# DixianZhu/deBWT

Measured on NVIDIA B200. Metric: bwt_build_throughput, higher is better.
Workload: dtype u64

## Files before the change

debwt_b200/csrc/api.cu:

```cuda
#include <algorithm>
#include <cstring>
#include <map>
#include <mutex>
#include <string>
#include <tuple>
#include <vector>

#include "../../include/debwt_b200.h"
#include "../../include/debwt_b200_dev.h"
#include "radix_sort.cuh"
#include "stages.cuh"
#include "special.cuh"
#include "ctx.cuh"
#include "dist_kernels.cuh"

namespace debwt {

static thread_local std::string g_err;
unsigned g_launches = 0;
unsigned long long g_launches_total = 0;
void set_error(const std::string& msg) { g_err = msg; }

#define FAIL(msg)            \
    do {                     \
// ... 298 lines not shown
    mark();

    u64 *d_ka = nullptr, *d_kb = nullptr;
    if (dalloc(pool, &d_ka, nk + 2) || dalloc(pool, &d_kb, nk + 2)) return -1;
    if (k_extract(d_text, n, d_seps, R, d_ka, st)) return -1;
    mark();

    void* d_sortws = nullptr;
    if (pool.alloc(&d_sortws, sort_workspace_bytes(nk, c->sort_cfg))) return -1;
    SortWorkspace ws;
    sort_workspace_bind(ws, d_sortws, nk, c->sort_cfg);
    int sweeps = 0;
    ws.ev_sweep_begin = c->ev[11]; ws.ev_sweep_end = c->ev[12]; ws.sweeps_out = &sweeps;
    const unsigned launches_before_sort = g_launches;
    u64* d_keys = nullptr;
    KeyIndex ki;
    ki.bits = key_index_bits(nk);
    if (dalloc(pool, &ki.idx, (1ull << ki.bits) + 2) || k_key_index_init(ki, st)) return -1;
    bool index_marked = false;
    ws.key_index = ki.idx; ws.key_index_bits = ki.bits; ws.key_index_done = &index_marked;
    const bool text_hist = text_digit_hist_applies(n, R);
    if (text_hist && (radix_sort_clear(ws, st) || k_text_digit_hist(d_text, n, d_seps, R, ws.hist, st))) return -1;
    if (radix_sort_u64(d_ka, d_kb, nk, ws, st, &d_keys, text_hist)) return -1;
    S.sort_launches = g_launches - launches_before_sort;
    S.sort_sweeps = (u32)sweeps;
    pool.adopt(d_keys == d_ka ? d_kb : d_ka, (nk + 2) * 8);
    pool.adopt(d_sortws, sort_workspace_bytes(nk, c->sort_cfg));
    u32 h_err[2] = {0, 0};
    CUDA_TRY(cudaMemcpyAsync(h_err, d_err, 8, cudaMemcpyDeviceToHost, st));
    mark();

    u16* d_gmask = nullptr;
    if (dalloc(pool, &d_gmask, nk + 2)) return -1;
    CUDA_TRY(cudaMemsetAsync(d_gmask, 0, (nk + 2) * 2, st));
    if (k_key_index_finish(d_keys, nk, ki, index_marked, st)) return -1;
    if (k_mark_edges(d_keys, nk, ki, d_gmask, st)) return -1;
    if (k_mark_heads_tails(d_text, d_seps, R, d_keys, nk, ki, d_gmask, st)) return -1;
    void* d_brws = nullptr; u64* d_tot = nullptr;
    if (pool.alloc(&d_brws, branch_workspace_bytes(nk)) || dalloc(pool, &d_tot, 4)) return -1;
    if (k_branch_count(d_keys, nk, d_gmask, true, d_brws, d_tot, st)) return -1;
    u64 h_tot[2] = {0, 0};
    CUDA_TRY(cudaMemcpyAsync(h_tot, d_tot, 16, cudaMemcpyDeviceToHost, st));
    CUDA_TRY(cudaStreamSynchronize(st));
    if (h_err[0]) FAIL(c->resolve_ambiguous ? "input contains a symbol that is neither a base nor an IUPAC ambiguity code"
                                            : "input contains a symbol other than A, C, G, T (either case)");
    if (h_err[1] != R) FAIL("input contains '#' or '$' inside a record (they are reserved for the record separators)");
    BranchTable bt;
    bt.n_branch = h_tot[0]; bt.n_blue = h_tot[1];
    S.n_branch = bt.n_branch; S.n_blue = bt.n_blue;
    {
        int bits = 8;
        while (bits < 27 && (1ull << bits) < 2 * bt.n_branch) ++bits;
        bt.bits = bits;
    }
    if (dalloc(pool, &bt.kmer, bt.n_branch + 1) || dalloc(pool, &bt.head, bt.n_branch + 1) ||
        dalloc(pool, &bt.blue, bt.n_branch + 2) || dalloc(pool, &bt.cursor, bt.n_branch + 1) ||
        dalloc(pool, &bt.bidx, BranchTable::index_words(bt.bits)))
        return -1;
    CUDA_TRY(cudaMemsetAsync(bt.cursor, 0, (bt.n_branch + 1) * 4, st));
    if (k_branch_write(d_keys, nk, d_gmask, d_brws, bt, st)) return -1;
    {
        const u32 m32 = (u32)bt.n_blue;
        CUDA_TRY(cudaMemcpyAsync(bt.blue + bt.n_branch, &m32, 4, cudaMemcpyHostToDevice, st));
    }
    if (k_branch_index(bt, st)) return -1;
    int id_bits = 1;
    while (id_bits < 64 && (bt.n_branch >> id_bits)) ++id_bits;
    const bool group_by_sort = id_bits <= 28 && n < (1ull << 32) && bt.n_blue > 1 &&
                               c->blue_grouping == 2;
    bt.hbits = BranchTable::hash_bits(bt.n_branch);
    bt.hmode = group_by_sort ? 0 : 1;
    if (dalloc(pool, &bt.hslots, 1ull << bt.hbits) || k_branch_hash(bt, st)) return -1;
    mark();
// ... 422 lines not shown
    if (s.get(&d_k, n + 2) || s.get(&d_km, n + 2) || s.get(&d_ct, n + 2) || s.get(&d_tot, 2)) return -1;
    CUDA_TRY(cudaMalloc(&d_ws, rle_workspace_bytes(n)));
    s.ptrs.push_back(d_ws);
    CUDA_TRY(cudaMemcpyAsync(d_k, sorted, n * 8, cudaMemcpyHostToDevice, s.st));
    if (k_rle(d_k, n, d_km, d_ct, d_ws, d_tot, s.st)) return -1;
    u64 d = 0;
    CUDA_TRY(cudaMemcpyAsync(&d, d_tot, 8, cudaMemcpyDeviceToHost, s.st));
    CUDA_TRY(cudaStreamSynchronize(s.st));
    CUDA_TRY(cudaMemcpyAsync(kmers_out, d_km, d * 8, cudaMemcpyDeviceToHost, s.st));
    CUDA_TRY(cudaMemcpyAsync(counts_out, d_ct, d * 8, cudaMemcpyDeviceToHost, s.st));
    CUDA_TRY(cudaStreamSynchronize(s.st));
    if (n_distinct_out) *n_distinct_out = d;
    return 0;
}

int debwt_k_group_masks(int device, const char* text, uint64_t n, const uint64_t* seps, uint64_t R, uint16_t* masks_out) {
    if (check_seps(seps, R, n)) return -1;
    Scratch s;
    if (open_scratch(s, device)) return -1;
    const u64 nk = n - 32 * R;
    u8* d_a; u64 *d_w, *d_s, *d_ka, *d_kb; u32* d_e; u16* d_g; void* d_ws;
    KeyIndex ki;
    ki.bits = key_index_bits(nk);
    if (s.get(&d_a, n + 64) || s.get(&d_w, text_words(n)) || s.get(&d_e, 4) || s.get(&d_s, R) || s.get(&d_ka, nk + 2) ||
        s.get(&d_kb, nk + 2) || s.get(&d_g, nk + 2) || s.get(&ki.idx, (1ull << ki.bits) + 2))
        return -1;
    CUDA_TRY(cudaMalloc(&d_ws, sort_workspace_bytes(nk, 0)));
    s.ptrs.push_back(d_ws);
    SortWorkspace ws;
    sort_workspace_bind(ws, d_ws, nk, 0);
    CUDA_TRY(cudaMemcpyAsync(d_a, text, n, cudaMemcpyHostToDevice, s.st));
    CUDA_TRY(cudaMemcpyAsync(d_s, seps, R * 8, cudaMemcpyHostToDevice, s.st));
    CUDA_TRY(cudaMemsetAsync(d_e, 0, 16, s.st));
    CUDA_TRY(cudaMemsetAsync(d_g, 0, (nk + 2) * 2, s.st));
    u64* d_keys = nullptr;
    if (k_pack(d_a, n, d_w, d_e, s.st) || k_extract(d_w, n, d_s, R, d_ka, s.st) ||
        radix_sort_u64(d_ka, d_kb, nk, ws, s.st, &d_keys) || k_build_key_index(d_keys, nk, ki, s.st) ||
        k_mark_edges(d_keys, nk, ki, d_g, s.st) || k_mark_heads_tails(d_w, d_s, R, d_keys, nk, ki, d_g, s.st) ||
        k_propagate(d_keys, nk, d_g, s.st))
        return -1;
    CUDA_TRY(cudaMemcpyAsync(masks_out, d_g, nk * 2, cudaMemcpyDeviceToHost, s.st));
    CUDA_TRY(cudaStreamSynchronize(s.st));
    return 0;
}


int debwt_k_codes(int device, const char* text, uint64_t n, const uint64_t* seps, uint64_t R, uint8_t* codes_out, uint64_t codes_cap,
                  uint64_t* n_codes_out, uint64_t* blue_head_out, uint64_t* blue_spindex_out, uint8_t* blue_prev_out, uint64_t blue_cap,
                  uint64_t* n_blue_out) {
    debwt_ctx* c = nullptr;
    if (debwt_create(&c, device)) return -1;
    c->cap.on = true;
    int rc = debwt_set_text(c, text, n, seps, R);
    if (!rc) rc = debwt_build(c, 32);
    if (!rc) {
        const auto& q = c->cap;
        if (n_codes_out) *n_codes_out = q.n_codes;
        if (n_blue_out) *n_blue_out = q.blue.size();
        if (q.n_codes > codes_cap || q.blue.size() > blue_cap) { set_error("debwt_k_codes: output buffers too small"); rc = -1; }
    }
    if (!rc) {
        const auto& q = c->cap;
        for (u64 i = 0; i < q.n_codes; ++i) {
            u8 code = (u8)((q.codes[i >> 5] >> (2 * (31 - (i & 31)))) & 3ull);
            if ((q.sep[i >> 5] >> (i & 31)) & 1u) code = i == q.dollar_index ? 5 : 4;
            codes_out[i] = code;
        }
        for (u64 b = 0; b < q.seg_kmer.size(); ++b)
            for (u32 e = q.seg_off[b]; e < q.seg_off[b + 1]; ++e) {
                blue_head_out[e] = q.seg_head[b];
                blue_spindex_out[e] = q.blue[e] >> 4;
                blue_prev_out[e] = (u8)(q.blue[e] & 15ull);
// ... 105 lines not shown
```

debwt_b200/csrc/stages.cu:

```cuda
#include "stages.cuh"

#include <cstdlib>
#include "special.cuh"
#include "stages_dev.cuh"
#include "dist_kernels.cuh"

namespace debwt {

namespace {

constexpr int TPB = 256;
inline unsigned grid_for(u64 work, int per_block) { return (unsigned)((work + per_block - 1) / per_block); }

constexpr int SCAN_ITEMS = 16;
constexpr int SCAN_TILE = TPB * SCAN_ITEMS;

template <bool POPC>
__device__ __forceinline__ u32 scan_f(u32 v) { return POPC ? (u32)__popc(v) : v; }

template <bool POPC>
__global__ void __launch_bounds__(TPB) scan_reduce_kernel(const u32* __restrict__ in, u64 m, u32* __restrict__ part) {
    __shared__ u32 sm[40];
    const u64 base = (u64)blockIdx.x * SCAN_TILE;
    u32 s = 0;
// ... 348 lines not shown
    void* scan_ws = p;
    p += (scan_workspace_bytes(nt) + 7) & ~(size_t)7;
    u64* starts = reinterpret_cast<u64*>(p);
    rle_count_kernel<<<(unsigned)nt, TPB, 0, st>>>(sorted, n, tile_cnt);
    if (scan_exclusive_u32(tile_cnt, tile_ex, nt, false, scan_ws, d_total, st)) return -1;
    rle_write_kernel<<<(unsigned)nt, TPB, 0, st>>>(sorted, n, tile_ex, kmers, starts);
    u64 d = 0;
    CUDA_TRY(cudaMemcpyAsync(&d, d_total, 8, cudaMemcpyDeviceToHost, st));
    CUDA_TRY(cudaStreamSynchronize(st));
    diff_kernel<<<grid_for(d, TPB), TPB, 0, st>>>(starts, d, n, counts);
    DEBWT_COUNT(3);
    CUDA_TRY(cudaGetLastError());
    return 0;
}

namespace {

__global__ void __launch_bounds__(TPB) key_index_mark_kernel(const u64* __restrict__ k, u64 n, KeyIndex ki) {
    const u64 i = (u64)blockIdx.x * TPB + threadIdx.x;
    if (i >= n) return;
    const int sh = 64 - ki.bits;
    const u64 cur = k[i] >> sh;
    if (i == 0 || (k[i - 1] >> sh) != cur) ki.idx[cur] = (u32)i;
}

__global__ void __launch_bounds__(TPB) key_index_fill_kernel(const u64* __restrict__ k, u64 n, KeyIndex ki) {
    const u64 t = (u64)blockIdx.x * TPB + threadIdx.x;
    const u64 nb = 1ull << ki.bits;
    if (t > nb) return;
    if (t == nb) { ki.idx[t] = (u32)n; return; }
    if (ki.idx[t] == 0xFFFFFFFFu) ki.idx[t] = (u32)lower_bound_u64(k, 0, n, t << (64 - ki.bits));
}

constexpr int ME_ROWS = 4;

__device__ __forceinline__ void edge_rows(const u64* __restrict__ k, u64 n, const KeyIndex& ki, u16* __restrict__ gmask, u64 base,
                                          u64 limit) {
    u64 key[ME_ROWS], lo[ME_ROWS], hi[ME_ROWS];
    bool act[ME_ROWS];
#pragma unroll
    for (int j = 0; j < ME_ROWS; ++j) {
        const u64 i = base + (u64)j * TPB;
        act[j] = i < limit;
        key[j] = act[j] ? k[i] : 0;
        if (act[j] && i > 0 && k[i - 1] == key[j]) act[j] = false;
    }
#pragma unroll
    for (int j = 0; j < ME_ROWS; ++j) {
        const u64 t = (key[j] << 2) >> (64 - ki.bits);
        lo[j] = act[j] ? ki.idx[t] : 0;
        hi[j] = act[j] ? ki.idx[t + 1] : 0;
    }
#pragma unroll
    for (int j = 0; j < ME_ROWS; ++j) {
        if (!act[j]) continue;
        const u64 q = key[j] << 2;
        const u64 hs = lower_bound_u64(k, lo[j], hi[j], q);
        if (hs < n && (k[hs] >> 2) == (q >> 2)) atomic_or_u16(gmask, hs, 1u << (u32)(key[j] >> 62));
    }
#pragma unroll
    for (int j = 0; j < ME_ROWS; ++j) {
        if (!act[j]) continue;
        const u64 i = base + (u64)j * TPB;
        atomic_or_u16(gmask, group_head(k, i), 1u << (GM_OUT_SHIFT + (u32)(key[j] & 3)));
    }
}

constexpr u64 ME_TILE = 8192;
constexpr u64 ME_CAP = 8 * ME_TILE;
struct EdgeRun { u64 begin, end; };

__global__ void __launch_bounds__(TPB) edge_bounds_kernel(const u64* __restrict__ k, u64 n, KeyIndex ki, u64 tiles,
                                                         u64* __restrict__ bounds) {
    const u64 x = (u64)blockIdx.x * TPB + threadIdx.x;
    if (x >= 4 * (tiles + 1)) return;
    const u32 c = (u32)(x / (tiles + 1));
    const u64 t = x % (tiles + 1);
    const u64 cbeg = ki.idx[(u64)c << (ki.bits - 2)];
    const u64 cend = (c == 3) ? n : (u64)ki.idx[(u64)(c + 1) << (ki.bits - 2)];
    const u64 a = t * ME_TILE;
    u64 r;
    if (a == 0) r = cbeg;
    else if (a >= n) r = cend;
    else {
        const u64 low = (k[a - 1] >> 2) + 1;
        r = (low >> 62) ? cend : indexed_lower_bound(k, ki, ((u64)c << 62) | low);
    }
    bounds[x] = r;
}

__global__ void __launch_bounds__(TPB) mark_edges_kernel(const u64* __restrict__ k, u64 n, KeyIndex ki, u16* __restrict__ gmask,
                                                        const u64* __restrict__ bounds, u64 tiles, EdgeRun* __restrict__ over,
                                                        u32* __restrict__ n_over) {
    const u32 c = blockIdx.x & 3u;
    const u64 tile = blockIdx.x >> 2;
    const u64 sb = bounds[c * (tiles + 1) + tile];
    u64 se = bounds[c * (tiles + 1) + tile + 1];
    if (se - sb > ME_CAP && se > sb) {
        if (threadIdx.x == 0) over[atomicAdd(n_over, 1u)] = EdgeRun{sb + ME_CAP, se};
        se = sb + ME_CAP;
    }
    for (u64 i0 = sb; i0 < se; i0 += (u64)TPB * ME_ROWS) edge_rows(k, n, ki, gmask, i0 + threadIdx.x, se);
}

__global__ void __launch_bounds__(TPB) mark_edges_over_kernel(const u64* __restrict__ k, u64 n, KeyIndex ki, u16* __restrict__ gmask,
                                                             const EdgeRun* __restrict__ over, const u32* __restrict__ n_over) {
    const u32 m = *n_over;
    for (u32 q = 0; q < m; ++q) {
        const EdgeRun r = over[q];
        for (u64 i0 = r.begin + (u64)blockIdx.x * (TPB * ME_ROWS); i0 < r.end; i0 += (u64)gridDim.x * (TPB * ME_ROWS))
            edge_rows(k, n, ki, gmask, i0 + threadIdx.x, r.end);
    }
}

__global__ void __launch_bounds__(TPB) mark_heads_tails_kernel(const u64* __restrict__ words, const u64* __restrict__ seps,
                                                              u64 n_rec, const u64* __restrict__ k, u64 n, KeyIndex ki,
                                                              u16* __restrict__ gmask) {
    const u64 r = (u64)blockIdx.x * TPB + threadIdx.x;
    if (r >= n_rec) return;
    const u64 start = r ? seps[r - 1] + 1 : 0;
    u64 x = text_window32(words, start) & ~3ull;
    u64 h = indexed_lower_bound(k, ki, x);
    if (h < n && (k[h] & ~3ull) == x) atomic_or_u16(gmask, h, GM_IN_SEP);
    x = text_window32(words, seps[r] - KNODE) & ~3ull;
    h = indexed_lower_bound(k, ki, x);
    if (h < n && (k[h] & ~3ull) == x) atomic_or_u16(gmask, h, GM_OUT_TAIL);
}

__global__ void __launch_bounds__(TPB) propagate_kernel(const u64* __restrict__ k, u64 n, u16* __restrict__ gmask) {
    const u64 i = (u64)blockIdx.x * TPB + threadIdx.x;
    if (i >= n || i == 0) return;
    if ((k[i - 1] >> 2) != (k[i] >> 2)) return;
    gmask[i] = gmask[group_head(k, i)];
}

constexpr int BR_ITEMS = 8;
constexpr int BR_TILE = TPB * BR_ITEMS;

template <bool WRITE, bool PROPAGATE>
__global__ void __launch_bounds__(TPB) branch_kernel(const u64* __restrict__ k, u64 n, u16* __restrict__ gmask,
                                                    u32* __restrict__ tile_nb, u32* __restrict__ tile_blue,
                                                    const u32* __restrict__ tile_nb_ex, const u32* __restrict__ tile_blue_ex,
                                                    u32* __restrict__ head_bits, BranchTable bt) {
    constexpr int NW = TPB / 32;
    __shared__ u32 s_cnt[BR_ITEMS * NW + 1], s_blue[BR_ITEMS * NW + 1];
    if (WRITE && tile_nb[blockIdx.x] == 0) return;
    const int lane = threadIdx.x & 31, warp = threadIdx.x >> 5;
// ... 59 lines not shown
            if (lane >= o) { ic += tc; ib += tb; }
        }
        const u32 ec = ic - (c0 + c1), eb = ib - (b0 + b1);
        s_cnt[2 * lane] = ec; s_cnt[2 * lane + 1] = ec + c0;
        s_blue[2 * lane] = eb; s_blue[2 * lane + 1] = eb + b0;
        if (lane == 31) {
            s_cnt[BR_ITEMS * NW] = ic; s_blue[BR_ITEMS * NW] = ib;
            if (!WRITE) { tile_nb[blockIdx.x] = ic; tile_blue[blockIdx.x] = ib; }
        }
    }
    if (!WRITE) return;
    __syncthreads();
    const u64 ob0 = tile_nb_ex[blockIdx.x];
    const u32 ol0 = tile_blue_ex[blockIdx.x];
#pragma unroll
    for (int j = 0; j < BR_ITEMS; ++j) {
        if (bal[j] == 0) continue;
        u32 inc = size[j];
#pragma unroll
        for (int o = 1; o < 32; o <<= 1) {
            const u32 t = __shfl_up_sync(0xffffffffu, inc, o);
            if (lane >= o) inc += t;
        }
        if (flags[j]) {
            const u64 i = base + (u64)j * TPB + threadIdx.x;
            const u64 ob = ob0 + s_cnt[j * NW + warp] + __popc(bal[j] & lt);
            bt.kmer[ob] = (k[i] & ~3ull) | (flags[j] & 3u);
            bt.head[ob] = (u32)i;
            bt.blue[ob] = ol0 + s_blue[j * NW + warp] + (inc - size[j]);
        }
    }
}

__global__ void __launch_bounds__(TPB) branch_index_kernel(BranchTable bt) {
    const u64 t = (u64)blockIdx.x * TPB + threadIdx.x;
    const u64 nb = 1ull << bt.bits;
    if (t > nb) return;
    bt.bidx[t] = (t == nb) ? (u32)bt.n_branch : (u32)lower_bound_u64(bt.kmer, 0, bt.n_branch, t << (64 - bt.bits));
}

__global__ void __launch_bounds__(TPB) branch_filter_kernel(BranchTable bt) {
    const u64 b = (u64)blockIdx.x * TPB + threadIdx.x;
    if (b >= bt.n_branch) return;
    const u64 f = bt.filter_of(bt.kmer[b] & ~3ull);
    atomicOr(bt.filter() + (f >> 5), 1u << (f & 31));
}

__global__ void __launch_bounds__(TPB) branch_hash_kernel(BranchTable bt) {
    const u64 b = (u64)blockIdx.x * TPB + threadIdx.x;
    if (b >= bt.n_branch) return;
    const u64 e = bt.kmer[b];
    const u64 mask = (1ull << bt.hbits) - 1;
    for (u64 h = bt.hash_of(e & ~3ull);; h = (h + 1) & mask) {
        unsigned long long* claim = reinterpret_cast<unsigned long long*>(&bt.hslots[h].x);
        if (atomicCAS(claim, 0ull, (unsigned long long)e) == 0ull) {
            bt.hslots[h].y = bt.hmode ? (u64)bt.blue[b] << 32 : b;
            return;
        }
    }
}

__global__ void __launch_bounds__(TPB) special_ins_kernel(const u64* __restrict__ k, u64 n, KeyIndex ki,
                                                         const u64* __restrict__ pads, u64 m, u64* __restrict__ ins) {
    const u64 t = (u64)blockIdx.x * TPB + threadIdx.x;
    if (t < m) ins[t] = indexed_upper_bound(k, ki, pads[t]);
}

}

int k_key_index_init(KeyIndex ki, cudaStream_t st) {
    CUDA_TRY(cudaMemsetAsync(ki.idx, 0xFF, ((1ull << ki.bits) + 1) * 4, st));
    return 0;
}

int k_key_index_finish(const u64* sorted, u64 n, KeyIndex ki, bool marked, cudaStream_t st) {
    if (n && !marked) {
        key_index_mark_kernel<<<grid_for(n, TPB), TPB, 0, st>>>(sorted, n, ki);
        DEBWT_COUNT(1);
    }
    key_index_fill_kernel<<<grid_for((1ull << ki.bits) + 1, TPB), TPB, 0, st>>>(sorted, n, ki);
    DEBWT_COUNT(1);
    CUDA_TRY(cudaGetLastError());
    return 0;
}

int k_build_key_index(const u64* sorted, u64 n, KeyIndex ki, cudaStream_t st) {
    if (k_key_index_init(ki, st)) return -1;
    return k_key_index_finish(sorted, n, ki, false, st);
}

int k_mark_edges(const u64* sorted, u64 n, KeyIndex ki, u16* gmask, cudaStream_t st) {
    if (n == 0) return 0;
    const u64 tiles = (n + ME_TILE - 1) / ME_TILE;
    const u64 cap = n / ME_CAP + 8;
    char* ws = nullptr;
    CUDA_TRY(cudaMallocAsync(reinterpret_cast<void**>(&ws), 16 + cap * sizeof(EdgeRun) + 4 * (tiles + 1) * 8, st));
    u32* n_over = reinterpret_cast<u32*>(ws);
    EdgeRun* over = reinterpret_cast<EdgeRun*>(ws + 16);
    u64* bounds = reinterpret_cast<u64*>(ws + 16 + cap * sizeof(EdgeRun));
    cudaMemsetAsync(n_over, 0, 16, st);
    edge_bounds_kernel<<<grid_for(4 * (tiles + 1), TPB), TPB, 0, st>>>(sorted, n, ki, tiles, bounds);
    mark_edges_kernel<<<(unsigned)(4 * tiles), TPB, 0, st>>>(sorted, n, ki, gmask, bounds, tiles, over, n_over);
    mark_edges_over_kernel<<<148 * 8, TPB, 0, st>>>(sorted, n, ki, gmask, over, n_over);
    DEBWT_COUNT(3);
    const cudaError_t e = cudaGetLastError();
    cudaFreeAsync(ws, st);
    if (e != cudaSuccess) { set_error(std::string("mark_edges: ") + cudaGetErrorString(e)); return -1; }
    return 0;
}

int k_mark_heads_tails(const u64* words, const u64* d_seps, u64 n_rec, const u64* sorted, u64 n, KeyIndex ki, u16* gmask,
                       cudaStream_t st) {
    mark_heads_tails_kernel<<<grid_for(n_rec, TPB), TPB, 0, st>>>(words, d_seps, n_rec, sorted, n, ki, gmask);
    DEBWT_COUNT(1);
    CUDA_TRY(cudaGetLastError());
    return 0;
}

int k_propagate(const u64* sorted, u64 n, u16* gmask, cudaStream_t st) {
    if (n == 0) return 0;
    propagate_kernel<<<grid_for(n, TPB), TPB, 0, st>>>(sorted, n, gmask);
    DEBWT_COUNT(1);
    CUDA_TRY(cudaGetLastError());
    return 0;
}

namespace {
struct BranchWs { u32 *nb, *blue, *nb_ex, *blue_ex, *head_bits; void* scan_ws; u64 nt; };
BranchWs branch_ws(void* workspace, u64 n) {
    BranchWs w;
    w.nt = (n + BR_TILE - 1) / BR_TILE;
    u32* p = reinterpret_cast<u32*>(workspace);
    w.nb = p; w.blue = p + w.nt; w.nb_ex = p + 2 * w.nt; w.blue_ex = p + 3 * w.nt;
    char* q = reinterpret_cast<char*>(p + 4 * w.nt);
    q += (8 - (reinterpret_cast<uintptr_t>(q) & 7)) & 7;
    w.scan_ws = q;
    q += (scan_workspace_bytes(w.nt + 1) + 15) & ~(size_t)15;
    w.head_bits = reinterpret_cast<u32*>(q);
    return w;
}
}

size_t branch_workspace_bytes(u64 n) {
    const u64 nt = (n + BR_TILE - 1) / BR_TILE + 1;
    return nt * 16 + 16 + scan_workspace_bytes(nt) + 32 + nt * (BR_TILE / 8);
}

int k_branch_count(const u64* sorted, u64 n, u16* gmask, bool propagate, void* workspace, u64* d_totals, cudaStream_t st) {
    BranchWs w = branch_ws(workspace, n);
    BranchTable none;
    if (propagate) branch_kernel<false, true><<<(unsigned)w.nt, TPB, 0, st>>>(sorted, n, gmask, w.nb, w.blue, nullptr, nullptr, w.head_bits, none);
    else branch_kernel<false, false><<<(unsigned)w.nt, TPB, 0, st>>>(sorted, n, gmask, w.nb, w.blue, nullptr, nullptr, w.head_bits, none);
    DEBWT_COUNT(1);
    if (scan_exclusive_u32(w.nb, w.nb_ex, w.nt, false, w.scan_ws, d_totals, st)) return -1;
    if (scan_exclusive_u32(w.blue, w.blue_ex, w.nt, false, w.scan_ws, d_totals + 1, st)) return -1;
    CUDA_TRY(cudaGetLastError());
    return 0;
}

int k_branch_write(const u64* sorted, u64 n, const u16* gmask, void* workspace, BranchTable bt, cudaStream_t st) {
    BranchWs w = branch_ws(workspace, n);
    branch_kernel<true, false><<<(unsigned)w.nt, TPB, 0, st>>>(sorted, n, const_cast<u16*>(gmask), w.nb, nullptr, w.nb_ex, w.blue_ex, w.head_bits, bt);
    DEBWT_COUNT(1);
    CUDA_TRY(cudaGetLastError());
    return 0;
}

int k_branch_index(BranchTable bt, cudaStream_t st) {
    branch_index_kernel<<<grid_for((1ull << bt.bits) + 1, TPB), TPB, 0, st>>>(bt);
    CUDA_TRY(cudaMemsetAsync(bt.filter(), 0, (1ull << (BranchTable::filter_bits(bt.bits) - 5)) * 4, st));
    if (bt.n_branch) branch_filter_kernel<<<grid_for(bt.n_branch, TPB), TPB, 0, st>>>(bt);
    DEBWT_COUNT(2);
    CUDA_TRY(cudaGetLastError());
    return 0;
}

int k_branch_hash(BranchTable bt, cudaStream_t st) {
    if (!bt.hslots) return 0;
    CUDA_TRY(cudaMemsetAsync(bt.hslots, 0, (1ull << bt.hbits) * sizeof(ulonglong2), st));
    if (bt.n_branch) branch_hash_kernel<<<grid_for(bt.n_branch, TPB), TPB, 0, st>>>(bt);
    DEBWT_COUNT(1);
    CUDA_TRY(cudaGetLastError());
    return 0;
}

namespace {
__global__ void __launch_bounds__(128) special_scan_kernel(const u64* __restrict__ words, const u64* __restrict__ seps,
                                                          u64 n_rec, const u64* __restrict__ k, u64 n_keys, KeyIndex ki,
                                                          SpecialInfo* __restrict__ out) {
    __shared__ u32 s_cnt;
    const u64 m = n_rec * 32;
    const u64 a = blockIdx.x;
    const u64 pa = seps[a >> 5] - (a & 31);
    if (threadIdx.x == 0) s_cnt = 0;
    __syncthreads();
    u32 cnt = 0;
    for (u64 b = threadIdx.x; b < m; b += blockDim.x) {
// ... 620 lines not shown
```

debwt_b200/csrc/stages.cuh:

```cuda
#pragma once
#include "common.cuh"

namespace debwt {

size_t scan_workspace_bytes(u64 m);
int scan_exclusive_u32(const u32* in, u32* out, u64 m, bool popc, void* workspace, u64* d_total, cudaStream_t st);

struct PackPolicy {
    bool resolve = false;
    u64 seed = 0;
    u64 pos_base = 0;
};
int k_pack(const u8* ascii, u64 n, u64* words, u32* d_err, cudaStream_t st, PackPolicy pol = PackPolicy());
inline u64 text_words(u64 n) { return (n + 32 + 31) / 32 + 1; }
int k_extract(const u64* words, u64 n, const u64* d_seps, u64 n_rec, u64* keys, cudaStream_t st);
int k_extract_slice(const u64* words, u64 n, u64 pos_lo, u64 pos_hi, const u64* d_seps, u64 n_rec, u64 idx_base, u64* keys,
                    cudaStream_t st);

bool text_digit_hist_applies(u64 n, u64 n_rec);
int k_text_digit_hist(const u64* words, u64 n, const u64* d_seps, u64 n_rec, u64* ghist, cudaStream_t st);

int k_rle(const u64* sorted, u64 n, u64* kmers, u64* counts, void* workspace, u64* d_total, cudaStream_t st);
size_t rle_workspace_bytes(u64 n);

struct KeyIndex {
    u32* idx = nullptr;
    int bits = 0;
};
inline int key_index_bits(u64 n) {
    int b = 8;
    while (b < 28 && (8ull << b) < n) ++b;
    return b;
}
int k_build_key_index(const u64* sorted, u64 n, KeyIndex ki, cudaStream_t st);
int k_key_index_init(KeyIndex ki, cudaStream_t st);
int k_key_index_finish(const u64* sorted, u64 n, KeyIndex ki, bool marked, cudaStream_t st);
__host__ __device__ __forceinline__ u64 indexed_lower_bound(const u64* __restrict__ k, const KeyIndex& ki, u64 q) {
    const u64 t = q >> (64 - ki.bits);
    return lower_bound_u64(k, ki.idx[t], ki.idx[t + 1], q);
}
__host__ __device__ __forceinline__ u64 indexed_upper_bound(const u64* __restrict__ k, const KeyIndex& ki, u64 q) {
    const u64 t = q >> (64 - ki.bits);
    return upper_bound_u64(k, ki.idx[t], ki.idx[t + 1], q);
}

int k_mark_edges(const u64* sorted, u64 n, KeyIndex ki, u16* gmask, cudaStream_t st);
int k_mark_heads_tails(const u64* words, const u64* d_seps, u64 n_rec, const u64* sorted, u64 n, KeyIndex ki, u16* gmask,
                       cudaStream_t st);
int k_propagate(const u64* sorted, u64 n, u16* gmask, cudaStream_t st);

struct BranchTable {
    u64 n_branch = 0;
    u64 n_blue = 0;
    u64* kmer = nullptr;
    u32* head = nullptr;
    u32* blue = nullptr;
    u32* cursor = nullptr;
    u32* bidx = nullptr;
    int bits = 0;
    ulonglong2* hslots = nullptr;
    int hbits = 0;
    int hmode = 0;
    __host__ __device__ static int hash_bits(u64 n_branch) { int b = 10; while (b < 40 && (1ull << b) < 3 * n_branch) ++b; return b; }
    __host__ __device__ u64 hash_of(u64 x) const { return ((x >> 2) * 0x9E3779B97F4A7C15ull) >> (64 - hbits); }
    __host__ __device__ u64 filter_of(u64 x) const { return ((x >> 2) * 0x9E3779B97F4A7C15ull) >> (64 - filter_bits(bits)); }
    __host__ __device__ static int filter_bits(int bits) { return bits + 3 < 30 ? bits + 3 : 30; }
    __host__ __device__ static u64 index_words(int bits) { return (1ull << bits) + 2 + (1ull << (filter_bits(bits) - 5)); }
    __host__ __device__ u32* filter() const { return bidx + (1ull << bits) + 2; }
};
size_t branch_workspace_bytes(u64 n);
int k_branch_count(const u64* sorted, u64 n, u16* gmask, bool propagate, void* workspace, u64* d_totals, cudaStream_t st);
int k_branch_write(const u64* sorted, u64 n, const u16* gmask, void* workspace, BranchTable bt, cudaStream_t st);
int k_branch_index(BranchTable bt, cudaStream_t st);
int k_branch_hash(BranchTable bt, cudaStream_t st);

int k_special_insertion(const u64* sorted, u64 n, KeyIndex ki, const u64* pads, u64 m, u64* ins, cudaStream_t st);

int k_flag_positions(const u64* words, u64 n, const u64* d_seps, u64 n_rec, BranchTable bt, u32* mo_bits, u64* blue,
                     cudaStream_t st);
int k_flag_positions_keys(const u64* words, u64 n, const u64* d_seps, u64 n_rec, BranchTable bt, int shift, u32* mo_bits,
                          u64* bkeys, u64* d_counter, cudaStream_t st);
int k_blue_keys_fix(u64* bkeys, u64 m, const u32* mo_bits, const u32* word_prefix, cudaStream_t st);
int k_blue_keys_strip(u64* bkeys, u64 m, cudaStream_t st);
int k_blue_fix_interleaved(u64* blue, u64 m, const u32* mo_bits, const u32* word_prefix, u64 n_words, u64* scratch, cudaStream_t st);
int k_patch_bits(u32* mo_bits, const u64* positions, u64 m, cudaStream_t st);
int k_emit_codes(const u64* words, u64 n, const u32* mo_bits, const u32* word_prefix, u64* sp_codes, cudaStream_t st);
int k_mark_sep_codes(const u32* mo_bits, const u32* word_prefix, const u64* positions, u64 m, u32* sp_sep,
                     u64* d_code_index_out, cudaStream_t st);
int k_blue_fix(u64* blue, u64 m, const u32* mo_bits, const u32* word_prefix, cudaStream_t st);

struct SpView {
    const u64* codes;
    const u32* sep;
    u64 dollar_index;
    u64 n_codes;
    const u32* sep_sum = nullptr;
};
int k_sort_blue(u64* blue, BranchTable bt, SpView sp, u32* d_work , cudaStream_t st);

int k_fill_case2(const u16* gmask, u64 n_keys, u64 n, const u64* spec_rows, u64 m, u64* bwt, cudaStream_t st);
int k_emit_blue(const u64* blue, BranchTable bt, const u64* spec_ins, u64 m, u64* bwt, u64* sharp_rows,
                u32* d_sharp_count, u64* dollar_row, cudaStream_t st);
int k_emit_special(const u64* spec_rows, const u8* spec_chr, u64 m, u64* bwt, cudaStream_t st);

}
// ... 1 lines not shown
```

Measured before the change: 9023.

## Fuse edge marking, head/tail flags and branch counting into tiled classify kernel

Replaces the separate mask memset, mark_edges (bounds, per-tile and overflow kernels), mark_heads_tails and branch_count propagate passes with one tile-based classify kernel. It stages each 4096-key tile in shared memory, resolves group heads with ballots and a warp prefix scan, and does the predecessor-edge lookups by searching within shared memory instead of through global atomics. Per-record separator flags come from a small pre-kernel, and cross-tile groups are handled with precomputed boundary info. This is meant to cut global atomics, redundant passes over the sorted keys and launch count. In exchange it adds considerable complexity and a large dynamic shared-memory footprint, and long runs that span tiles fall back to global searches.

```diff
diff --git a/debwt_b200/csrc/api.cu b/debwt_b200/csrc/api.cu
--- a/debwt_b200/csrc/api.cu
+++ b/debwt_b200/csrc/api.cu
@@ -354,13 +354,12 @@
 
     u16* d_gmask = nullptr;
     if (dalloc(pool, &d_gmask, nk + 2)) return -1;
-    CUDA_TRY(cudaMemsetAsync(d_gmask, 0, (nk + 2) * 2, st));
     if (k_key_index_finish(d_keys, nk, ki, index_marked, st)) return -1;
-    if (k_mark_edges(d_keys, nk, ki, d_gmask, st)) return -1;
-    if (k_mark_heads_tails(d_text, d_seps, R, d_keys, nk, ki, d_gmask, st)) return -1;
-    void* d_brws = nullptr; u64* d_tot = nullptr;
-    if (pool.alloc(&d_brws, branch_workspace_bytes(nk)) || dalloc(pool, &d_tot, 4)) return -1;
-    if (k_branch_count(d_keys, nk, d_gmask, true, d_brws, d_tot, st)) return -1;
+    void* d_brws = nullptr; void* d_clws = nullptr; u64* d_tot = nullptr;
+    if (pool.alloc(&d_brws, branch_workspace_bytes(nk)) || pool.alloc(&d_clws, classify_workspace_bytes(nk)) ||
+        dalloc(pool, &d_tot, 4))
+        return -1;
+    if (k_classify(d_text, d_seps, R, d_keys, nk, ki, d_gmask, d_clws, d_brws, d_tot, st)) return -1;
     u64 h_tot[2] = {0, 0};
     CUDA_TRY(cudaMemcpyAsync(h_tot, d_tot, 16, cudaMemcpyDeviceToHost, st));
     CUDA_TRY(cudaStreamSynchronize(st));
@@ -849,12 +848,13 @@
     CUDA_TRY(cudaMemcpyAsync(d_a, text, n, cudaMemcpyHostToDevice, s.st));
     CUDA_TRY(cudaMemcpyAsync(d_s, seps, R * 8, cudaMemcpyHostToDevice, s.st));
     CUDA_TRY(cudaMemsetAsync(d_e, 0, 16, s.st));
-    CUDA_TRY(cudaMemsetAsync(d_g, 0, (nk + 2) * 2, s.st));
+    u8 *d_brws, *d_clws;
+    u64* d_tot;
+    if (s.get(&d_brws, branch_workspace_bytes(nk)) || s.get(&d_clws, classify_workspace_bytes(nk)) || s.get(&d_tot, 4)) return -1;
     u64* d_keys = nullptr;
     if (k_pack(d_a, n, d_w, d_e, s.st) || k_extract(d_w, n, d_s, R, d_ka, s.st) ||
         radix_sort_u64(d_ka, d_kb, nk, ws, s.st, &d_keys) || k_build_key_index(d_keys, nk, ki, s.st) ||
-        k_mark_edges(d_keys, nk, ki, d_g, s.st) || k_mark_heads_tails(d_w, d_s, R, d_keys, nk, ki, d_g, s.st) ||
-        k_propagate(d_keys, nk, d_g, s.st))
+        k_classify(d_w, d_s, R, d_keys, nk, ki, d_g, d_clws, d_brws, d_tot, s.st))
         return -1;
     CUDA_TRY(cudaMemcpyAsync(masks_out, d_g, nk * 2, cudaMemcpyDeviceToHost, s.st));
     CUDA_TRY(cudaStreamSynchronize(s.st));
diff --git a/debwt_b200/csrc/stages.cu b/debwt_b200/csrc/stages.cu
--- a/debwt_b200/csrc/stages.cu
+++ b/debwt_b200/csrc/stages.cu
@@ -404,87 +404,6 @@
     if (ki.idx[t] == 0xFFFFFFFFu) ki.idx[t] = (u32)lower_bound_u64(k, 0, n, t << (64 - ki.bits));
 }
 
-constexpr int ME_ROWS = 4;
-
-__device__ __forceinline__ void edge_rows(const u64* __restrict__ k, u64 n, const KeyIndex& ki, u16* __restrict__ gmask, u64 base,
-                                          u64 limit) {
-    u64 key[ME_ROWS], lo[ME_ROWS], hi[ME_ROWS];
-    bool act[ME_ROWS];
-#pragma unroll
-    for (int j = 0; j < ME_ROWS; ++j) {
-        const u64 i = base + (u64)j * TPB;
-        act[j] = i < limit;
-        key[j] = act[j] ? k[i] : 0;
-        if (act[j] && i > 0 && k[i - 1] == key[j]) act[j] = false;
-    }
-#pragma unroll
-    for (int j = 0; j < ME_ROWS; ++j) {
-        const u64 t = (key[j] << 2) >> (64 - ki.bits);
-        lo[j] = act[j] ? ki.idx[t] : 0;
-        hi[j] = act[j] ? ki.idx[t + 1] : 0;
-    }
-#pragma unroll
-    for (int j = 0; j < ME_ROWS; ++j) {
-        if (!act[j]) continue;
-        const u64 q = key[j] << 2;
-        const u64 hs = lower_bound_u64(k, lo[j], hi[j], q);
-        if (hs < n && (k[hs] >> 2) == (q >> 2)) atomic_or_u16(gmask, hs, 1u << (u32)(key[j] >> 62));
-    }
-#pragma unroll
-    for (int j = 0; j < ME_ROWS; ++j) {
-        if (!act[j]) continue;
-        const u64 i = base + (u64)j * TPB;
-        atomic_or_u16(gmask, group_head(k, i), 1u << (GM_OUT_SHIFT + (u32)(key[j] & 3)));
-    }
-}
-
-constexpr u64 ME_TILE = 8192;
-constexpr u64 ME_CAP = 8 * ME_TILE;
-struct EdgeRun { u64 begin, end; };
-
-__global__ void __launch_bounds__(TPB) edge_bounds_kernel(const u64* __restrict__ k, u64 n, KeyIndex ki, u64 tiles,
-                                                         u64* __restrict__ bounds) {
-    const u64 x = (u64)blockIdx.x * TPB + threadIdx.x;
-    if (x >= 4 * (tiles + 1)) return;
-    const u32 c = (u32)(x / (tiles + 1));
-    const u64 t = x % (tiles + 1);
-    const u64 cbeg = ki.idx[(u64)c << (ki.bits - 2)];
-    const u64 cend = (c == 3) ? n : (u64)ki.idx[(u64)(c + 1) << (ki.bits - 2)];
-    const u64 a = t * ME_TILE;
-    u64 r;
-    if (a == 0) r = cbeg;
-    else if (a >= n) r = cend;
-    else {
-        const u64 low = (k[a - 1] >> 2) + 1;
-        r = (low >> 62) ? cend : indexed_lower_bound(k, ki, ((u64)c << 62) | low);
-    }
-    bounds[x] = r;
-}
-
-__global__ void __launch_bounds__(TPB) mark_edges_kernel(const u64* __restrict__ k, u64 n, KeyIndex ki, u16* __restrict__ gmask,
-                                                        const u64* __restrict__ bounds, u64 tiles, EdgeRun* __restrict__ over,
-                                                        u32* __restrict__ n_over) {
-    const u32 c = blockIdx.x & 3u;
-    const u64 tile = blockIdx.x >> 2;
-    const u64 sb = bounds[c * (tiles + 1) + tile];
-    u64 se = bounds[c * (tiles + 1) + tile + 1];
-    if (se - sb > ME_CAP && se > sb) {
-        if (threadIdx.x == 0) over[atomicAdd(n_over, 1u)] = EdgeRun{sb + ME_CAP, se};
-        se = sb + ME_CAP;
-    }
-    for (u64 i0 = sb; i0 < se; i0 += (u64)TPB * ME_ROWS) edge_rows(k, n, ki, gmask, i0 + threadIdx.x, se);
-}
-
-__global__ void __launch_bounds__(TPB) mark_edges_over_kernel(const u64* __restrict__ k, u64 n, KeyIndex ki, u16* __restrict__ gmask,
-                                                             const EdgeRun* __restrict__ over, const u32* __restrict__ n_over) {
-    const u32 m = *n_over;
-    for (u32 q = 0; q < m; ++q) {
-        const EdgeRun r = over[q];
-        for (u64 i0 = r.begin + (u64)blockIdx.x * (TPB * ME_ROWS); i0 < r.end; i0 += (u64)gridDim.x * (TPB * ME_ROWS))
-            edge_rows(k, n, ki, gmask, i0 + threadIdx.x, r.end);
-    }
-}
-
 __global__ void __launch_bounds__(TPB) mark_heads_tails_kernel(const u64* __restrict__ words, const u64* __restrict__ seps,
                                                               u64 n_rec, const u64* __restrict__ k, u64 n, KeyIndex ki,
                                                               u16* __restrict__ gmask) {
@@ -610,6 +529,246 @@
     }
 }
 
+constexpr int CL_TPB = 256;
+constexpr int CL_ROWS = 16;
+constexpr int CL_TILE = CL_TPB * CL_ROWS;
+constexpr int CL_SEGS = CL_TILE / 32;
+constexpr int CL_SRC = 16;
+constexpr u64 CL_CHUNK = (u64)CL_TPB * CL_SRC;
+constexpr size_t CL_SMEM = CL_TILE * 8 + CL_TILE * 4 + CL_SEGS * 4 * 2;
+static_assert(CL_TILE == 2 * BR_TILE && CL_TPB == TPB, "a classify tile holds two branch tiles");
+static_assert(CL_TILE < (1 << 13), "tile-local group ends are kept in bits 16..28 of the shared mask");
+
+__global__ void __launch_bounds__(TPB) sep_flags_kernel(const u64* __restrict__ words, const u64* __restrict__ seps, u64 n_rec,
+                                                       const u64* __restrict__ k, u64 n, KeyIndex ki, u32* __restrict__ sepf) {
+    const u64 r = (u64)blockIdx.x * TPB + threadIdx.x;
+    if (r >= n_rec) return;
+    const u64 start = r ? seps[r - 1] + 1 : 0;
+    u64 x = text_window32(words, start) & ~3ull;
+    u64 h = indexed_lower_bound(k, ki, x);
+    if (h < n && (k[h] & ~3ull) == x) atomicOr(sepf + (h >> 4), 1u << (2 * (u32)(h & 15)));
+    x = text_window32(words, seps[r] - KNODE) & ~3ull;
+    h = indexed_lower_bound(k, ki, x);
+    if (h < n && (k[h] & ~3ull) == x) atomicOr(sepf + (h >> 4), 2u << (2 * (u32)(h & 15)));
+}
+
+__global__ void __launch_bounds__(TPB) classify_bounds_kernel(const u64* __restrict__ k, u64 n, KeyIndex ki, u64 tiles,
+                                                             const u32* __restrict__ sepf, u64* __restrict__ bounds,
+                                                             u8* __restrict__ cross) {
+    const u64 x = (u64)blockIdx.x * TPB + threadIdx.x;
+    if (x >= tiles * 12) return;
+    const u64 t = x / 12;
+    const u32 s = (u32)(x % 12);
+    const u64 base = t * CL_TILE;
+    if (s < 8) {
+        const u64 last = (base + CL_TILE < n ? base + CL_TILE : n) - 1;
+        const u64 q = ((u64)(s & 3) << 62) | (k[s < 4 ? base : last] >> 2);
+        bounds[t * 8 + s] = s < 4 ? indexed_lower_bound(k, ki, q) : indexed_upper_bound(k, ki, q);
+        return;
+    }
+    const u32 y = s - 8;
+    u32 v = 0;
+    const u64 key = k[base];
+    if (t > 0 && (k[base - 1] >> 2) == (key >> 2)) {
+        const u64 q = (key & ~3ull) | y;
+        const u64 h = indexed_lower_bound(k, ki, q);
+        if (h < n && k[h] == q) v = 1u << y;
+        if (y == 0) v |= ((sepf[h >> 4] >> (2 * (u32)(h & 15))) & 3u) << 4;
+    }
+    cross[t * 4 + y] = (u8)v;
+}
+
+__device__ __forceinline__ u32 cross_mask(u32 v) {
+    v |= v >> 16;
+    v |= v >> 8;
+    return ((v & 15u) << GM_OUT_SHIFT) | ((v & 16u) ? GM_IN_SEP : 0u) | ((v & 32u) ? GM_OUT_TAIL : 0u);
+}
+
+__device__ __forceinline__ u32 smem_lower_bound(const u64* __restrict__ a, u32 lo, u32 hi, u64 q) {
+    while (lo < hi) {
+        const u32 mid = (lo + hi) >> 1;
+        if (a[mid] < q) lo = mid + 1; else hi = mid;
+    }
+    return lo;
+}
+
+__device__ __forceinline__ u32 slot_of(u32 i, const u32* __restrict__ s_hb, const int* __restrict__ s_pre) {
+    const u32 m = s_hb[i >> 5] & (0xFFFFFFFFu >> (31 - (i & 31)));
+    return m ? (i & ~31u) + 31 - __clz(m) : (u32)s_pre[i >> 5];
+}
+
+__global__ void __launch_bounds__(CL_TPB, 4) classify_kernel(const u64* __restrict__ k, u64 n, const u64* __restrict__ bounds,
+                                                            const u32* __restrict__ cross, const u32* __restrict__ sepf,
+                                                            u16* __restrict__ gmask, u32* __restrict__ tile_nb,
+                                                            u32* __restrict__ tile_blue, u32* __restrict__ head_bits, u64 br_tiles) {
+    extern __shared__ u64 s_k[];
+    u32* s_gm = reinterpret_cast<u32*>(s_k + CL_TILE);
+    u32* s_hb = s_gm + CL_TILE;
+    int* s_pre = reinterpret_cast<int*>(s_hb + CL_SEGS);
+    __shared__ u64 s_run[8];
+    __shared__ u32 s_sep[CL_TILE / 16], s_cross[2];
+    __shared__ u32 s_cnt[2][CL_TPB / 32], s_blue[2][CL_TPB / 32];
+    const int lane = threadIdx.x & 31, warp = threadIdx.x >> 5;
+    const u64 base = (u64)blockIdx.x * CL_TILE;
+    const u32 tv = (u32)(n - base < (u64)CL_TILE ? n - base : (u64)CL_TILE);
+    {
+        u64 key[CL_ROWS];
+#pragma unroll
+        for (int r = 0; r < CL_ROWS; ++r) {
+            const u32 i = r * CL_TPB + threadIdx.x;
+            key[r] = i < tv ? k[base + i] : ~0ull;
+        }
+        static_assert(CL_TILE / 16 == CL_TPB, "one word of flags per thread");
+        s_sep[threadIdx.x] = threadIdx.x * 16 < tv ? sepf[base / 16 + threadIdx.x] : 0u;
+        if (threadIdx.x < 8) s_run[threadIdx.x] = bounds[(u64)blockIdx.x * 8 + threadIdx.x];
+        if (threadIdx.x == 8) s_cross[0] = cross[blockIdx.x];
+        if (threadIdx.x == 9) s_cross[1] = base + tv < n ? cross[blockIdx.x + 1] : 0u;
+#pragma unroll
+        for (int r = 0; r < CL_ROWS; ++r) s_k[r * CL_TPB + threadIdx.x] = key[r];
+    }
+    const u64 left = base ? k[base - 1] : 0;
+    const u64 right = base + tv < n ? k[base + tv] : ~0ull;
+    __syncthreads();
+    const bool cross_right = base + tv < n && (right >> 2) == (s_k[tv - 1] >> 2);
+#pragma unroll 4
+    for (int r = 0; r < CL_ROWS; ++r) {
+        const u32 i = r * CL_TPB + threadIdx.x;
+        const u64 key = s_k[i];
+        const u64 prev = i ? s_k[i - 1] : left;
+        const bool head = i < tv && (base + i == 0 || (prev >> 2) != (key >> 2));
+        const u32 hb = __ballot_sync(0xffffffffu, head);
+        if (lane == 0) s_hb[i >> 5] = hb;
+        u32 m = 0;
+        if (head) {
+            const u32 f = (s_sep[i >> 4] >> (2 * (i & 15))) & 3u;
+            m = (1u << (GM_OUT_SHIFT + (u32)(key & 3))) | ((f & 1u) ? GM_IN_SEP : 0u) | ((f & 2u) ? GM_OUT_TAIL : 0u);
+        }
+        s_gm[i] = m;
+    }
+    __syncthreads();
+    if (warp == 0) {
+        static_assert(CL_SEGS == 4 * 32, "four warp rows per lane");
+        int last[4], m = -1;
+#pragma unroll
+        for (int j = 0; j < 4; ++j) {
+            const u32 hb = s_hb[4 * lane + j];
+            if (hb) m = (4 * lane + j) * 32 + 31 - __clz(hb);
+            last[j] = m;
+        }
+        int inc = m;
+#pragma unroll
+        for (int o = 1; o < 32; o <<= 1) {
+            const int t = __shfl_up_sync(0xffffffffu, inc, o);
+            if (lane >= o && t > inc) inc = t;
+        }
+        int ex = __shfl_up_sync(0xffffffffu, inc, 1);
+        if (lane == 0) ex = -1;
+#pragma unroll
+        for (int j = 0; j < 4; ++j) {
+            s_pre[4 * lane + j] = ex < 0 ? 0 : ex;
+            if (last[j] > ex) ex = last[j];
+        }
+    }
+    __syncthreads();
+#pragma unroll 4
+    for (int r = 0; r < CL_ROWS; ++r) {
+        const u32 i = r * CL_TPB + threadIdx.x;
+        if (i >= tv) break;
+        const u32 slot = slot_of(i, s_hb, s_pre);
+        const u64 key = s_k[i];
+        u32 add = (slot != i) ? 1u << (GM_OUT_SHIFT + (u32)(key & 3)) : 0u;
+        if (i + 1 == tv || (s_k[i + 1] >> 2) != (key >> 2)) add |= (i + 1) << 16;
+        if (i == 0 && slot == 0 && base && (left >> 2) == (key >> 2)) add |= cross_mask(s_cross[0]);
+        if (i + 1 == tv && cross_right) add |= cross_mask(s_cross[1]);
+        if (add) atomicOr(s_gm + slot, add);
+    }
+    u64 o1, o2, o3, len;
+    {
+        const u64 l0 = s_run[4] - s_run[0], l1 = s_run[5] - s_run[1], l2 = s_run[6] - s_run[2], l3 = s_run[7] - s_run[3];
+        o1 = l0; o2 = o1 + l1; o3 = o2 + l2; len = o3 + l3;
+    }
+    auto at = [&](u64 v) -> u64 {
+        return v < o1 ? s_run[0] + v : v < o2 ? s_run[1] + (v - o1) : v < o3 ? s_run[2] + (v - o2) : s_run[3] + (v - o3);
+    };
+    auto run_end = [&](u64 v) -> u64 {
+        return v < o1 ? s_run[4] : v < o2 ? s_run[5] : v < o3 ? s_run[6] : s_run[7];
+    };
+    for (u64 p0 = 0; p0 < len;) {
+        const u64 p1 = p0 + CL_CHUNK < len ? p0 + CL_CHUNK : len;
+        const u64 a = p0 + (u64)threadIdx.x * CL_SRC;
+        u64 src[CL_SRC];
+#pragma unroll
+        for (int j = 0; j < CL_SRC; ++j) src[j] = (a + j < p1) ? k[at(a + j)] : ~0ull;
+        u64 next = p1;
+        if (p1 < len && p1 != o1 && p1 != o2 && p1 != o3) {
+            const u64 x = at(p1), se = run_end(p1), v = k[x - 1];
+            if (k[x] == v) {
+                u64 lo = x, step = 1;
+                while (lo + step < se && k[lo + step] == v) { lo += step; step <<= 1; }
+                next = p1 + (upper_bound_u64(k, lo + 1, lo + step < se ? lo + step : se, v) - x);
+            }
+        }
+        if (a < p1) {
+            u64 q = src[0] << 2;
+            u32 p = smem_lower_bound(s_k, 0, tv, q);
+            if (p < tv && (s_k[p] >> 2) == (q >> 2)) atomicOr(s_gm + p, 1u << (u32)(src[0] >> 62));
+#pragma unroll
+            for (int j = 1; j < CL_SRC; ++j) {
+                if (a + j >= p1) break;
+                if (src[j] == src[j - 1]) continue;
+                const u64 q2 = src[j] << 2;
+                if (q2 < q) p = smem_lower_bound(s_k, 0, tv, q2);
+                else
+                    for (int w = 0; p < tv && s_k[p] < q2; ++w, ++p)
+                        if (w == 8) { p = smem_lower_bound(s_k, p, tv, q2); break; }
+                q = q2;
+                if (p < tv && (s_k[p] >> 2) == (q >> 2)) atomicOr(s_gm + p, 1u << (u32)(src[j] >> 62));
+            }
+        }
+        p0 = next;
+    }
+    __syncthreads();
+    u32 cnt0 = 0, cnt1 = 0, blue0 = 0, blue1 = 0;
+#pragma unroll 4
+    for (int r = 0; r < CL_ROWS; ++r) {
+        const u32 i = r * CL_TPB + threadIdx.x;
+        u32 flag = 0, size = 0;
+        if (i < tv) {
+            const u32 m = s_gm[slot_of(i, s_hb, s_pre)];
+            gmask[base + i] = (u16)m;
+            if ((s_hb[i >> 5] >> lane) & 1u) {
+                const u32 f = (gm_multi_out(m) ? 1u : 0u) | (gm_multi_in(m) ? 2u : 0u);
+                flag = f;
+                if (f & 2u) {
+                    const u32 end = (m >> 16) & 0x1FFFu;
+                    size = (end == tv && cross_right) ? (u32)(group_end(k, n, base + i) - (base + i)) : end - i;
+                }
+            }
+        }
+        const u32 bal = __ballot_sync(0xffffffffu, flag != 0);
+        const u64 row = (base + (u64)r * CL_TPB) / 32 + warp;
+        if (lane == 0 && row * 32 < br_tiles * BR_TILE) head_bits[row] = bal;
+        if (bal) {
+#pragma unroll
+            for (int o = 16; o; o >>= 1) size += __shfl_xor_sync(0xffffffffu, size, o);
+        }
+        if (r < CL_ROWS / 2) { cnt0 += __popc(bal); blue0 += size; }
+        else { cnt1 += __popc(bal); blue1 += size; }
+    }
+    if (lane == 0) {
+        s_cnt[0][warp] = cnt0; s_cnt[1][warp] = cnt1;
+        s_blue[0][warp] = blue0; s_blue[1][warp] = blue1;
+    }
+    __syncthreads();
+    if (threadIdx.x < 2) {
+        const u64 bt = (u64)blockIdx.x * 2 + threadIdx.x;
+        u32 c = 0, b = 0;
+#pragma unroll
+        for (int w = 0; w < CL_TPB / 32; ++w) { c += s_cnt[threadIdx.x][w]; b += s_blue[threadIdx.x][w]; }
+        if (bt < br_tiles) { tile_nb[bt] = c; tile_blue[bt] = b; }
+    }
+}
+
 __global__ void __launch_bounds__(TPB) branch_index_kernel(BranchTable bt) {
     const u64 t = (u64)blockIdx.x * TPB + threadIdx.x;
     const u64 nb = 1ull << bt.bits;
@@ -665,26 +824,6 @@
 int k_build_key_index(const u64* sorted, u64 n, KeyIndex ki, cudaStream_t st) {
     if (k_key_index_init(ki, st)) return -1;
     return k_key_index_finish(sorted, n, ki, false, st);
-}
-
-int k_mark_edges(const u64* sorted, u64 n, KeyIndex ki, u16* gmask, cudaStream_t st) {
-    if (n == 0) return 0;
-    const u64 tiles = (n + ME_TILE - 1) / ME_TILE;
-    const u64 cap = n / ME_CAP + 8;
-    char* ws = nullptr;
-    CUDA_TRY(cudaMallocAsync(reinterpret_cast<void**>(&ws), 16 + cap * sizeof(EdgeRun) + 4 * (tiles + 1) * 8, st));
-    u32* n_over = reinterpret_cast<u32*>(ws);
-    EdgeRun* over = reinterpret_cast<EdgeRun*>(ws + 16);
-    u64* bounds = reinterpret_cast<u64*>(ws + 16 + cap * sizeof(EdgeRun));
-    cudaMemsetAsync(n_over, 0, 16, st);
-    edge_bounds_kernel<<<grid_for(4 * (tiles + 1), TPB), TPB, 0, st>>>(sorted, n, ki, tiles, bounds);
-    mark_edges_kernel<<<(unsigned)(4 * tiles), TPB, 0, st>>>(sorted, n, ki, gmask, bounds, tiles, over, n_over);
-    mark_edges_over_kernel<<<148 * 8, TPB, 0, st>>>(sorted, n, ki, gmask, over, n_over);
-    DEBWT_COUNT(3);
-    const cudaError_t e = cudaGetLastError();
-    cudaFreeAsync(ws, st);
-    if (e != cudaSuccess) { set_error(std::string("mark_edges: ") + cudaGetErrorString(e)); return -1; }
-    return 0;
 }
 
 int k_mark_heads_tails(const u64* words, const u64* d_seps, u64 n_rec, const u64* sorted, u64 n, KeyIndex ki, u16* gmask,
@@ -741,6 +880,42 @@
     branch_kernel<true, false><<<(unsigned)w.nt, TPB, 0, st>>>(sorted, n, const_cast<u16*>(gmask), w.nb, nullptr, w.nb_ex, w.blue_ex, w.head_bits, bt);
     DEBWT_COUNT(1);
     CUDA_TRY(cudaGetLastError());
+    return 0;
+}
+
+namespace {
+struct ClassifyWs { u64* bounds; u32* sepf; u8* cross; u64 tiles; };
+ClassifyWs classify_ws(void* workspace, u64 n) {
+    ClassifyWs w;
+    w.tiles = (n + CL_TILE - 1) / CL_TILE;
+    w.bounds = reinterpret_cast<u64*>(workspace);
+    w.sepf = reinterpret_cast<u32*>(w.bounds + 8 * w.tiles);
+    w.cross = reinterpret_cast<u8*>(w.sepf + (n + 15) / 16 + 1);
+    return w;
+}
+}
+
+size_t classify_workspace_bytes(u64 n) {
+    const u64 tiles = (n + CL_TILE - 1) / CL_TILE;
+    return tiles * 64 + ((n + 15) / 16 + 1) * 4 + tiles * 4 + 64;
+}
+
+int k_classify(const u64* words, const u64* d_seps, u64 n_rec, const u64* sorted, u64 n, KeyIndex ki, u16* gmask,
+               void* cl_workspace, void* br_workspace, u64* d_totals, cudaStream_t st) {
+    BranchWs b = branch_ws(br_workspace, n);
+    if (n == 0) return scan_exclusive_u32(b.nb, b.nb_ex, 0, false, b.scan_ws, d_totals, st) ||
+                       scan_exclusive_u32(b.blue, b.blue_ex, 0, false, b.scan_ws, d_totals + 1, st);
+    ClassifyWs w = classify_ws(cl_workspace, n);
+    CUDA_TRY(cudaMemsetAsync(w.sepf, 0, ((n + 15) / 16 + 1) * 4, st));
+    if (n_rec) sep_flags_kernel<<<grid_for(n_rec, TPB), TPB, 0, st>>>(words, d_seps, n_rec, sorted, n, ki, w.sepf);
+    classify_bounds_kernel<<<grid_for(w.tiles * 12, TPB), TPB, 0, st>>>(sorted, n, ki, w.tiles, w.sepf, w.bounds, w.cross);
+    CUDA_TRY(cudaFuncSetAttribute(classify_kernel, cudaFuncAttributeMaxDynamicSharedMemorySize, (int)CL_SMEM));
+    classify_kernel<<<(unsigned)w.tiles, CL_TPB, CL_SMEM, st>>>(sorted, n, w.bounds, reinterpret_cast<const u32*>(w.cross), w.sepf,
+                                                             gmask, b.nb, b.blue, b.head_bits, b.nt);
+    DEBWT_COUNT(3);
+    CUDA_TRY(cudaGetLastError());
+    if (scan_exclusive_u32(b.nb, b.nb_ex, b.nt, false, b.scan_ws, d_totals, st)) return -1;
+    if (scan_exclusive_u32(b.blue, b.blue_ex, b.nt, false, b.scan_ws, d_totals + 1, st)) return -1;
     return 0;
 }
 
diff --git a/debwt_b200/csrc/stages.cuh b/debwt_b200/csrc/stages.cuh
--- a/debwt_b200/csrc/stages.cuh
+++ b/debwt_b200/csrc/stages.cuh
@@ -44,7 +44,6 @@
     return upper_bound_u64(k, ki.idx[t], ki.idx[t + 1], q);
 }
 
-int k_mark_edges(const u64* sorted, u64 n, KeyIndex ki, u16* gmask, cudaStream_t st);
 int k_mark_heads_tails(const u64* words, const u64* d_seps, u64 n_rec, const u64* sorted, u64 n, KeyIndex ki, u16* gmask,
                        cudaStream_t st);
 int k_propagate(const u64* sorted, u64 n, u16* gmask, cudaStream_t st);
@@ -71,6 +70,9 @@
 size_t branch_workspace_bytes(u64 n);
 int k_branch_count(const u64* sorted, u64 n, u16* gmask, bool propagate, void* workspace, u64* d_totals, cudaStream_t st);
 int k_branch_write(const u64* sorted, u64 n, const u16* gmask, void* workspace, BranchTable bt, cudaStream_t st);
+size_t classify_workspace_bytes(u64 n);
+int k_classify(const u64* words, const u64* d_seps, u64 n_rec, const u64* sorted, u64 n, KeyIndex ki, u16* gmask,
+               void* cl_workspace, void* br_workspace, u64* d_totals, cudaStream_t st);
 int k_branch_index(BranchTable bt, cudaStream_t st);
 int k_branch_hash(BranchTable bt, cudaStream_t st);
 
```

Result: slower. 8658 (median of 6 runs) (-4.0%).
